# Jabruson/FDN-TIP2025

Hardware: AMD Instinct MI355X
Metric: images/sec, FDN (LPNet->FDN forward) 1280x720 bs=8 fp32 (higher is better)
Workload: dtype f32

## Files before the change

### fdn-tip2025_amd/basicsr/models/archs/FDN_arch.py

```python
import numbers

import numpy as np
import torch
import torch.nn as nn
import torch.nn.functional as F
from einops import rearrange

import fdn_hip
from fdn_hip import ACT_LEAKY, ACT_NONE, ACT_SIGMOID, ops


_Cache = ops.WeightCache


def _w(p):
    return p.detach()


class WithBias_LayerNorm(nn.Module):

    def __init__(self, dim):
        super().__init__()
        self.weight = nn.Parameter(torch.ones(dim))
        self.bias = nn.Parameter(torch.zeros(dim))
# ... 196 lines not shown
    def forward(self, enc, dnc, x_high=None, x_high_p=None, x_img=None):
        n = self.n_feat
        x = ops.conv1x1([enc, dnc], _w(self.conv.weight), _w(self.conv.bias), want_stats=True, cache=(self._c, "c1"))
        x = self.att_channel((x, x_high, x_high_p, x_img))[0]
        wf = self._c.get("w", [self.conv2.weight], lambda: self.conv2.weight.detach()[:n] + self.conv2.weight.detach()[n:])
        bf = self._c.get("b", [self.conv2.bias], lambda: self.conv2.bias.detach()[:n] + self.conv2.bias.detach()[n:])
        return ops.conv1x1(x, wf, bf, cache=(self._c, "c2"), want_stats=True)


class OverlapPatchEmbed(nn.Module):
    def __init__(self, in_c=3, embed_dim=48, bias=False):
        super().__init__()
        self.proj = nn.Conv2d(in_c, embed_dim, kernel_size=3, stride=1, padding=1, bias=bias)

    def forward(self, x):
        return ops.conv2d(x, _w(self.proj.weight), pad=1)


class Downsample(nn.Module):

    def __init__(self, n_feat):
        super().__init__()
        self.body = nn.Sequential(nn.Identity(), nn.Conv2d(n_feat, n_feat * 2, 3, stride=1, padding=1, bias=False))

    def forward(self, x):
        return ops.conv2d(ops.resample(x, ops.RS_BILINEAR_HALF), _w(self.body[1].weight), pad=1)


class Upsample(nn.Module):

    def __init__(self, n_feat):
        super().__init__()
        self.body = nn.Sequential(nn.Identity(), nn.Conv2d(n_feat, n_feat // 2, 3, stride=1, padding=1, bias=False))
        self._c = _Cache()

    def forward(self, x):
        if ops.UPCONV_GATHER:
            return ops.upsample_conv3x3(x, _w(self.body[1].weight), cache=(self._c, "up"))
        return ops.conv2d(ops.resample(x, ops.RS_BILINEAR_X2), _w(self.body[1].weight), pad=1)


class FDformer(nn.Module):

    def __init__(self, inp_channels=3, out_channels=3, dim=48, num_blocks=[6, 6, 12, 8], num_refinement_blocks=4,
                 ffn_expansion_factor=3, bias=False):
        super().__init__()

        def stage(d, n, enc):
            return nn.Sequential(*[TransformerBlock(dim=d, ffn_expansion_factor=ffn_expansion_factor, bias=bias, att=True,
                                                    mode=1 if enc else 2, use_light=enc, use_img=enc) for _ in range(n)])

        self.patch_embed = OverlapPatchEmbed(inp_channels, dim)
        self.encoder_level1 = stage(dim, num_blocks[0], True)
        self.down1_2 = Downsample(dim)
        self.encoder_level2 = stage(dim * 2, num_blocks[1], True)
        self.down2_3 = Downsample(dim * 2)
        self.encoder_level3 = stage(dim * 4, num_blocks[2], True)
        self.decoder_level3 = stage(dim * 4, num_blocks[2], False)
        self.up3_2 = Upsample(dim * 4)
        self.reduce_chan_level2 = nn.Conv2d(dim * 4, dim * 2, kernel_size=1, bias=bias)
        self.decoder_level2 = stage(dim * 2, num_blocks[1], False)
        self.up2_1 = Upsample(dim * 2)
# ... 8 lines not shown
                x_high32=None, x1=None, x2=None, x3=None):
        e1 = self.encoder_level1((self.patch_embed(inp_img), x_high1, x_high12, x1))[0]
        e2 = self.encoder_level2((self.down1_2(e1), x_high2, x_high22, x2))[0]
        e3 = self.encoder_level3((self.down2_3(e2), x_high3, x_high32, x3))[0]
        d3 = self.decoder_level3((e3, x_high3, x_high32, x3))[0]
        d2 = self.fuse2(self.up3_2(d3), e2, x_high2, x_high22, x2)
        d2 = self.decoder_level2((d2, x_high2, x_high22, x2))[0]
        d1 = self.fuse1(self.up2_1(d2), e1, x_high1, x_high12, x1)
        d1 = self.decoder_level1((d1, x_high1, x_high12, x1))[0]
        d1 = self.refinement((d1, x_high1, x_high12, x1))[0]
        res = inp_img if ori_img is None else ori_img
        return ops.conv2d(d1, _w(self.output.weight), pad=1, res=res)


class BasicConv(nn.Module):
    def __init__(self, in_channel, out_channel, kernel_size, stride, bias=True, relu=True, transpose=False):
        super().__init__()
        self.k, self.stride, self.relu, self.transpose = kernel_size, stride, relu, transpose
        if transpose:
            conv = nn.ConvTranspose2d(in_channel, out_channel, kernel_size, padding=kernel_size // 2 - 1, stride=stride, bias=bias)
        else:
            conv = nn.Conv2d(in_channel, out_channel, kernel_size, padding=kernel_size // 2, stride=stride, bias=bias)
        self.main = nn.Sequential(conv)

    def forward(self, x, res=None, res_before_act=False, act=None, post_add=0.0):
        c = self.main[0]
        a = (ACT_LEAKY if self.relu else ACT_NONE) if act is None else act
        if self.transpose:
            return ops.conv_transpose4x4s2(x, _w(c.weight), _w(c.bias), a)
        if self.k == 1 and self.stride == 1:
            return ops.conv1x1(x, _w(c.weight), _w(c.bias), act=a)
        return ops.conv2d(x, _w(c.weight), _w(c.bias), stride=self.stride, pad=self.k // 2, act=a, res=res,
                          res_before_act=res_before_act, post_add=post_add)


class FAM(nn.Module):
    def __init__(self, channel):
        super().__init__()
        self.merge1 = nn.Conv2d(channel * 2, channel, kernel_size=1)
        self.merge2 = nn.Conv2d(channel, channel, kernel_size=3, stride=1, padding=1)

    def forward(self, x1, x2):
        t = ops.conv1x1([x1, x2], _w(self.merge1.weight), _w(self.merge1.bias))
        return ops.conv2d(t, _w(self.merge2.weight), _w(self.merge2.bias), pad=1)


def _mlp2(seq, x):
    t = ops.conv1x1(x, _w(seq[0].weight), _w(seq[0].bias), act=ACT_LEAKY)
    return ops.conv1x1(t, _w(seq[2].weight), _w(seq[2].bias))


def _spectral_mlps(y, process1, process2, H, W):
    z = ops.rfft_rows(y)
    mag, pha = ops.fft_cols_fwd(z, True, True, rd_before=False, fix_real=True)
    if ops.SPECTRAL_MLP_FUSED and mag.shape[1] in ops.SPECTRAL_MLP_C:
        ops.spectral_mlp2(mag, pha, _w(process1[0].weight), _w(process1[0].bias), _w(process1[2].weight), _w(process1[2].bias),
                          _w(process2[0].weight), _w(process2[0].bias), _w(process2[2].weight), _w(process2[2].bias), slope=0.1)
    else:
        mag = _mlp2(process1, mag)
        pha = _mlp2(process2, pha)
    return ops.fft_cols_inv_polar(mag, pha, H, W // 2 + 1)


class FreBlock(nn.Module):
    def __init__(self, nc):
        super().__init__()
        self.fpre = nn.Conv2d(nc, nc, 1, 1, 0)
# ... 26 lines not shown
        self.fourier_out = nn.Conv2d(out_nc, out_nc, 3, 1, 1)
        self._c = _Cache()

    def forward(self, x1, x2, x4):
        return self._rest(ops.conv1x1([x1, x2, x4], _w(self.fpre[0].weight), _w(self.fpre[0].bias)))

    def forward_multires(self, same, up1, up2):
        wfull, bias = _w(self.fpre[0].weight), _w(self.fpre[0].bias)
        n = wfull.shape[0]
        ks = sum(t.shape[1] for t in same)
        k1 = 0 if up1 is None else up1.shape[1]
        w2 = wfull.reshape(n, -1)
        parts = self._c.get("split", [self.fpre[0].weight], lambda: (w2[:, :ks].contiguous(), w2[:, ks:ks + k1].contiguous(), w2[:, ks + k1:].contiguous()))
        acc = ops.conv1x1(up2, parts[2])
        if up1 is not None:
            acc = ops.conv1x1(up1, parts[1], res=ops.resample(acc, ops.RS_NEAREST_X2))
        return self._rest(ops.conv1x1(same, parts[0], bias, res=ops.resample(acc, ops.RS_NEAREST_X2)))

    def _rest(self, y):
        H, W = y.shape[-2:]
        y = ops.dw1x1_pad1(y, _w(self.fpre[1].weight), _w(self.fpre[1].bias))
        zz = _spectral_mlps(y, self.process1, self.process2, H, W)
        xo = ops.irfft_rows(zz, H, W, 2.0 / (H * W))
        return ops.conv2d(xo, _w(self.fourier_out.weight), _w(self.fourier_out.bias), pad=1)


class MAR_archa(nn.Module):
    def __init__(self, use_ratio=True, block=None, apply_ratio=True):
        super().__init__()
        ProcessBlock_ = ProcessBlock if block is None else block
        self.use_ratio = use_ratio
        self.apply_ratio = apply_ratio
        c = 12
        self.Encoder = nn.ModuleList([ProcessBlock_(c), ProcessBlock_(c * 2), ProcessBlock_(c * 4)])
        self.Decoder = nn.ModuleList([ProcessBlock_(c * 4), ProcessBlock_(c * 2), ProcessBlock_(c)])
        self.Convs = nn.ModuleList([BasicConv(c * 4, c * 2, 1, 1, relu=True), BasicConv(c * 2, c, 1, 1, relu=True)])
        self.ConvsOut = nn.ModuleList([BasicConv(c * 4, 3, 3, 1, relu=False), BasicConv(c * 2, 3, 3, 1, relu=False)])
        self.AFFs = nn.ModuleList([fourier_fuse(c * 7, c), fourier_fuse(c * 7, c * 2)])
        self.FAM1 = FAM(c * 4)
        self.f1 = nn.Sequential(nn.Conv2d(3 * 16, c * 4, 1, 1, 0), ProcessBlock_(c * 4))
        self.f2 = nn.Sequential(nn.Conv2d(3 * 4, c * 2, 1, 1, 0), ProcessBlock_(c * 2))
        self.f3 = nn.Sequential(nn.Conv2d(3, c, 1, 1, 0), ProcessBlock_(c))
        self.f3_down = BasicConv(c, c * 2, 3, 2, relu=True)
        self.f2_down = BasicConv(c * 2, c * 4, 3, 2, relu=True)
        self.f2_up = BasicConv(c * 4, c * 2, 4, 2, relu=True, transpose=True)
        self.f3_up = BasicConv(c * 2, c, 4, 2, relu=True, transpose=True)
        self.out = BasicConv(c, 3, 3, 1, relu=False)
# ... 88 lines not shown
```

### fdn-tip2025_amd/basicsr/models/archs/LPNet_arch.py

```python
import torch
import torch.nn as nn
import torch.nn.functional as F
from einops import rearrange

from fdn_hip import ACT_NONE, ACT_RELU, ACT_SIGMOID, ops

from .FDN_arch import _Cache, _w

try:
    from torchvision import transforms
except Exception:
    class _Grayscale:
        def __init__(self, num_output_channels=1):
            self.n = num_output_channels

        def __call__(self, x):
            r, g, b = x.unbind(dim=-3)
            y = (0.2989 * r + 0.587 * g + 0.114 * b).unsqueeze(-3)
            return y if self.n == 1 else y.expand(*x.shape)

    class _Compose:
        def __init__(self, ts):
            self.ts = ts

# ... 23 lines not shown
    def __init__(self, in_channels, filters, stride=1, is_1x1conv=False):
        super().__init__()
        f1, f2, f3 = filters
        self.stride = stride
        self.is_1x1conv = is_1x1conv
        self.conv1 = nn.Sequential(nn.Conv2d(in_channels, f1, 1, stride=stride, bias=False), nn.BatchNorm2d(f1), nn.ReLU())
        self.conv2 = nn.Sequential(nn.Conv2d(f1, f2, 3, stride=1, padding=1, bias=False), nn.BatchNorm2d(f2), nn.ReLU())
        self.conv3 = nn.Sequential(nn.Conv2d(f2, f3, 1, stride=1, bias=False), nn.BatchNorm2d(f3))
        if is_1x1conv:
            self.shortcut = nn.Sequential(nn.Conv2d(in_channels, f3, 1, stride=stride, bias=False), nn.BatchNorm2d(f3))
        self.se = nn.Sequential(nn.AdaptiveAvgPool2d((1, 1)), nn.Conv2d(f3, f3 // 16, 1), nn.ReLU(),
                                nn.Conv2d(f3 // 16, f3, 1), nn.Sigmoid())
        self._c = _Cache()

    def _pw(self, x, seq, name, act, stride):
        w, b = _fold(seq[0], seq[1], self._c, name)
        if stride == 1:
            return ops.conv1x1(x, w, b, act=act)
        return ops.conv2d(x, w, b, stride=stride, pad=0, act=act)

    def forward(self, x):
        y = self._pw(x, self.conv1, "c1", ACT_RELU, self.stride)
        w2, b2 = _fold(self.conv2[0], self.conv2[1], self._c, "c2")
        y = ops.conv2d(y, w2, b2, stride=1, pad=1, act=ACT_RELU)
        y = self._pw(y, self.conv3, "c3", ACT_NONE, 1)
        g = ops.global_avgpool(y)
        g = ops.conv1x1(g, _w(self.se[1].weight), _w(self.se[1].bias), act=ACT_RELU)
        g = ops.conv1x1(g, _w(self.se[3].weight), _w(self.se[3].bias), act=ACT_SIGMOID)
        sc = self._pw(x, self.shortcut, "sc", ACT_NONE, self.stride) if self.is_1x1conv else x
        return ops.se_apply(y, g, sc)


class I_predict_net(nn.Module):

    def __init__(self, c=16):
        super().__init__()
        self.conv1 = nn.Sequential(nn.Conv2d(3, c, kernel_size=7, stride=2, padding=3, bias=False), nn.BatchNorm2d(c),
                                   nn.ReLU(), nn.AvgPool2d(kernel_size=3, stride=2, padding=1))
        self.conv2 = self._make_layer(c, (c, c, 2 * c), 3, 1)
        self.conv3 = self._make_layer(2 * c, (2 * c, 2 * c, 4 * c), 3, 2)
        self.conv4 = self._make_layer(4 * c, (4 * c, 4 * c, 8 * c), 6, 6)
        self.global_average_pool = nn.AdaptiveAvgPool2d((1, 1))
        self.fc = nn.Sequential(nn.Linear(8 * c, 8 * c))
        self.fc2 = nn.Sequential(nn.Linear(8 * c, 1))
        self.sigmoid = nn.Sigmoid()
        self.trans_gray = transforms.Compose([transforms.Grayscale(num_output_channels=1)])
        self._c = _Cache()
# ... 25 lines not shown
```

### fdn-tip2025_amd/csrc/conv3x3.hip

```cpp
#include "common.hpp"
#include <type_traits>

namespace {

constexpr int KC = 32;
using f32x16 = fdn_f32x16;

struct C3Args {
    const float* x; const float* w; const float* bias; const float* res; float* out;
    int B, Cin, H, W, Cout;
    int act, res_before_act; float post_add;
    int tiles_per_img, total_tiles;
    int n0, CoutT;
};

template <int MT, int NW>
__global__ __launch_bounds__(NW * 64, NW == 4 ? 2 : 1) void conv3x3_kernel(C3Args a) {
    extern __shared__ __attribute__((aligned(16))) float Wl[];
    constexpr int NT = NW * 64;
    constexpr int WS = MT * 32 + 1;
    constexpr int CH = KC * WS;
    constexpr int WPT = (KC * MT * 32) / NT;
    const int Cin = a.Cin, N = a.Cout, W = a.W, H = a.H;
    const int Ce = (Cin + 1) & ~1;
// ... 101 lines not shown
                            v = apply_act(v, a.act);
                            if (a.res && !a.res_before_act) v += bload(rr, voff, soff);
                            bstore(v + a.post_add, ro, voff, soff);
                        }
                }
#pragma unroll
                for (int m = 0; m < MT; ++m)
#pragma unroll
                    for (int r = 0; r < 16; ++r) acc[m][r] = 0.f;
            }
            if (nlive) w_stash((step + 1) & 1);
            __syncthreads();
            if (nlive && nc == 0) cur = nxt;
#pragma unroll
            for (int s = 0; s < 16; ++s) xa[s] = xb[s];
            tile = ntile; c = nc; live = nlive;
            ++step;
        }
    }
}

constexpr int TW = 32, CK = 8, HC = TW + 2;

template <int MT, int NW>
__global__ __launch_bounds__(NW * 64, (NW == 4 && MT == 1) ? 2 : 1) void conv3x3_split_kernel(C3Args a, int tiles_x, int tiles_y) {
    extern __shared__ __attribute__((aligned(16))) fdn_u32x4 smem4[];
    constexpr int NT = NW * 64, TH_ = 2 * NW, HR_ = TH_ + 2, NPOS = HR_ * HC;
    constexpr int N = MT * 32, KS5 = 5;
    constexpr int XB = 3 * NPOS, WB = KS5 * 3 * MT * 64;
    constexpr int XE = (NPOS + NT - 1) / NT;
    constexpr int WE = (N * 9 * CK + NT - 1) / NT;
    fdn_u32x4* Xs = smem4;
    fdn_u32x4* Ws = smem4 + 2 * XB;
    const int Cin = a.Cin, H = a.H, W = a.W;
    const unsigned P = (unsigned)H * W, P4 = P * 4u;
    const int tid = threadIdx.x, lane = tid & 63, wave = tid >> 6, kh = lane >> 5, ln = lane & 31;
    const int nchunk = Cin / CK;
    int b, y0, x0;
    {
        const unsigned T = (unsigned)(tiles_x * tiles_y) * a.B;
        const unsigned S0 = xcd_contiguous(blockIdx.x, gridDim.x);
        const unsigned grp = S0 / T, S = S0 - grp * T;
        a.n0 = (int)grp * N;
        const unsigned per = (unsigned)(tiles_x * tiles_y);
        b = (int)(S / per);
        const unsigned t = S - (unsigned)b * per;
        const int ty = (int)(t / (unsigned)tiles_x);
        y0 = ty * TH_;
        x0 = (int)(t - (unsigned)ty * tiles_x) * TW;
    }
    const int nvalid = min(N, a.CoutT - a.n0);
    unsigned xg[XE];
    int xl[XE];
#pragma unroll
    for (int i = 0; i < XE; ++i) {
        const int e = tid + NT * i, r = e / HC, c = e - r * HC;
        const int gy = y0 - 1 + r, gx = x0 - 1 + c;
        const bool in = e < NPOS, ok = in && gy >= 0 && gy < H && gx >= 0 && gx < W;
        xg[i] = ok ? (unsigned)(gy * W + gx) * 4u : 0x80000000u;
        xl[i] = in ? e : -1;
    }
    const rsrc_t rx = mk_rsrc(a.x + (long)b * Cin * P, (unsigned)Cin * P4);
    struct Stage { float xr[XE][CK], wr[WE]; };
    Stage stg[2];
    auto fetch = [&](int c, Stage& sg) __attribute__((always_inline)) {
        float (&xr)[XE][CK] = sg.xr;
        float (&wr)[WE] = sg.wr;
#pragma unroll
        for (int i = 0; i < XE; ++i)
#pragma unroll
            for (int ci = 0; ci < CK; ++ci) xr[i][ci] = bload(rx, xg[i], (unsigned)(c * CK + ci) * P4);
#pragma unroll
        for (int i = 0; i < WE; ++i) {
// ... 57 lines not shown
    auto chunk_step = [&](int c, Stage& mine, const Stage& nxt) __attribute__((always_inline)) {
        const bool more = c + 1 < nchunk;
        if (c + 2 < nchunk) fetch(c + 2, mine);
        const fdn_u32x4* xb = Xs + (c & 1) * XB;
        const fdn_u32x4* wb = Ws + (c & 1) * WB + lane;
#pragma unroll
        for (int s_ = 0; s_ < KS5; ++s_) {
            const fdn_u32x4 b0[3] = {xb[toff[s_]], xb[NPOS + toff[s_]], xb[2 * NPOS + toff[s_]]};
            const fdn_u32x4 b1[3] = {xb[toff[s_] + HC], xb[NPOS + toff[s_] + HC], xb[2 * NPOS + toff[s_] + HC]};
#pragma unroll
            for (int m = 0; m < MT; ++m) {
                const fdn_u32x4 av[3] = {wb[((s_ * 3 + 0) * MT + m) * 64], wb[((s_ * 3 + 1) * MT + m) * 64], wb[((s_ * 3 + 2) * MT + m) * 64]};
                acc[0][m] = fdn_mfma_split6(av, b0, acc[0][m]);
                acc[1][m] = fdn_mfma_split6(av, b1, acc[1][m]);
            }
        }
        if (more) stash((c + 1) & 1, nxt);
        __syncthreads();
    };
    for (int c = 0; c < nchunk; c += 2) {
        chunk_step(c, stg[0], stg[1]);
        if (c + 1 < nchunk) chunk_step(c + 1, stg[1], stg[0]);
    }
    const unsigned nb4 = (unsigned)nvalid * P4;
    const long obase = ((long)b * a.CoutT + a.n0) * P;
    const rsrc_t ro = mk_rsrc(a.out + obase, nb4);
    const rsrc_t rr = mk_rsrc(a.res ? a.res + obase : a.out, a.res ? nb4 : 0u);
    auto epilogue = [&](auto has_act) __attribute__((always_inline)) {
        const int act_ = decltype(has_act)::value ? a.act : (int)FDN_ACT_NONE;
#pragma unroll
        for (int st = 0; st < 2; ++st) {
            const int gy = y0 + row0 + st, gx = x0 + ln;
            const unsigned voff = (gy < H && gx < W) ? (4u * kh * P + (unsigned)(gy * W + gx)) * 4u : 0x80000000u;
#pragma unroll
            for (int m = 0; m < MT; ++m) {
                float rv[16];
                if (a.res) {
#pragma unroll
                    for (int r = 0; r < 16; ++r) {
                        const int nrow = m * 32 + (r & 3) + 8 * (r >> 2);
                        rv[r] = bload(rr, (nrow + 4 * kh < nvalid) ? voff : 0x80000000u, (unsigned)nrow * P4);
                    }
                }
#pragma unroll
                for (int r = 0; r < 16; ++r) {
                    const int nrow = m * 32 + (r & 3) + 8 * (r >> 2);
                    float v = acc[st][m][r];
                    if (a.bias) v += a.bias[a.n0 + min(nrow + 4 * kh, nvalid - 1)];
                    if (a.res && a.res_before_act) v += rv[r];
                    v = apply_act(v, act_);
                    if (a.res && !a.res_before_act) v += rv[r];
                    bstore(v + a.post_add, ro, (nrow + 4 * kh < nvalid) ? voff : 0x80000000u, (unsigned)nrow * P4);
                }
            }
        }
    };
    if (a.act == FDN_ACT_NONE) epilogue(std::false_type{}); else epilogue(std::true_type{});
}

template <int MT, int NW>
int launch_split(const C3Args& a, hipStream_t s) {
    constexpr int N = MT * 32, TH_ = 2 * NW;
    const size_t lds = 2UL * (3UL * (TH_ + 2) * HC + 5UL * 3 * MT * 64) * sizeof(fdn_u32x4);
    auto kern = conv3x3_split_kernel<MT, NW>;
    if (lds > 48 * 1024 && !fdn_allow_dynamic_lds(reinterpret_cast<const void*>(kern), lds)) return FDN_ERR_LAUNCH;
    const int tx = cdiv(a.W, TW), ty = cdiv(a.H, TH_);
    const long total = (long)tx * ty * a.B * cdiv(a.Cout, N);
    if (total > 0x7FFFFFFFL) return FDN_ERR_UNSUPPORTED;
    fdn_note_bf16_launch();
    hipLaunchKernelGGL(kern, dim3((unsigned)total), dim3(NW * 64), lds, s, a, tx, ty);
    return fdn_launch_status();
}

template <int MT, int NW>
int launch(C3Args a, hipStream_t s) {
    const size_t lds = 2UL * KC * (MT * 32 + 1) * sizeof(float);
    a.tiles_per_img = cdiv((long)a.H * a.W, NW * 32);
    a.total_tiles = a.B * a.tiles_per_img;
    auto kern = conv3x3_kernel<MT, NW>;
    const int grid = fdn_persistent_grid(kern, NW * 64, lds, a.total_tiles, {true, 0, 16, 0});
    if (grid < 0) return FDN_ERR_LAUNCH;
    hipLaunchKernelGGL(kern, dim3(grid), dim3(NW * 64), lds, s, a);
    return fdn_launch_status();
}

}

int fdn_conv3x3_mfma(const float* x, const float* w, const float* bias, const float* res, float* out, int B, int Cin, int H,
                     int W, int Cout, int act, int res_before_act, float post_add, hipStream_t s) {
    if (Cin < 2 || Cout < 8) return FDN_ERR_UNSUPPORTED;
    const unsigned long long P4 = 4ull * H * W;
    if ((unsigned long long)(Cin + 2) * P4 > 0xFFFFFFFFull || (unsigned long long)(Cout + 200) * P4 > 0xFFFFFFFFull)
        return FDN_ERR_UNSUPPORTED;
    C3Args a;
    a.x = x; a.w = w; a.bias = bias; a.res = res; a.out = out;
    a.B = B; a.Cin = Cin; a.H = H; a.W = W; a.Cout = Cout;
    a.act = act; a.res_before_act = res_before_act; a.post_add = post_add;
    a.tiles_per_img = a.total_tiles = 0;
    a.n0 = 0; a.CoutT = Cout;
    if (!fdn_matrix_pipe_f32() && Cin % CK == 0 && Cin >= 2 * CK && Cout >= 16)
        return Cout <= 32 ? launch_split<1, 4>(a, s) : launch_split<2, 8>(a, s);
    const int tiles = (Cout + 31) / 32;
    if (tiles == 1) return launch<1, 4>(a, s);
    if (tiles == 2) return launch<2, 4>(a, s);
    if (tiles == 3) return launch<3, 4>(a, s);
    return launch<4, 4>(a, s);
}
```

### fdn-tip2025_amd/fdn_hip/__init__.py

```python
import ctypes
import os

import torch

_HERE = os.path.dirname(os.path.abspath(__file__))
_LIB_PATH = os.path.join(_HERE, "libfdn_hip.so")
_lib = None

ACT_NONE, ACT_LEAKY, ACT_RELU, ACT_SIGMOID, ACT_GELU = 0, 1, 2, 3, 4
PRO_NONE, PRO_LN, PRO_LN3_GATE, PRO_LN_MULADD = 0, 1, 2, 3
EPI_NONE, EPI_RES, EPI_MULADD = 0, 1, 2

c_fp = ctypes.c_void_p


class Conv1x1Desc(ctypes.Structure):
    _fields_ = [
        ("x", c_fp * 3), ("xbs", ctypes.c_long * 3), ("kseg", ctypes.c_int * 3),
        ("w", c_fp), ("bias", c_fp), ("out", c_fp), ("obs", ctypes.c_long),
        ("B", ctypes.c_int), ("K", ctypes.c_int), ("N", ctypes.c_int), ("P", ctypes.c_int),
        ("pro", ctypes.c_int), ("ln_group", ctypes.c_int),
        ("stats", c_fp), ("gamma", c_fp), ("beta", c_fp), ("xb", c_fp), ("xbbs", ctypes.c_long),
        ("act", ctypes.c_int), ("epi", ctypes.c_int),
        ("res", c_fp), ("rbs", ctypes.c_long), ("mul", c_fp), ("add", c_fp), ("mbs", ctypes.c_long),
        ("vec4", ctypes.c_int), ("stats_out", c_fp), ("x_bf16", ctypes.c_int), ("out_bf16", ctypes.c_int), ("wpk", c_fp),
    ]


class FdnHipError(RuntimeError):
    pass


ABI_VERSION = 22
VIDEO_ABI_VERSION = 1
TEMPORAL_ABI_VERSION = 1
VMETRICS_ABI_VERSION = 1
ENSEMBLE_ABI_VERSION = 1


def lib_path():
    return _LIB_PATH


def lib():
    global _lib
    if _lib is None:
        if not os.path.isfile(_LIB_PATH):
            raise ImportError(
                f"{_LIB_PATH} not found: build it with fdn-tip2025_amd/build.sh (hipcc --offload-arch=gfx950). "
                "The FDN path has no CPU fallback.")
        _lib = ctypes.CDLL(_LIB_PATH)
        _declare(_lib)
        if _lib.fdn_abi_version() != ABI_VERSION:
            v = _lib.fdn_abi_version()
            _lib = None
            raise ImportError(f"{_LIB_PATH} has ABI version {v}, this binding needs {ABI_VERSION}: rebuild with build.sh")
        if _lib.fdn_video_abi_version() != VIDEO_ABI_VERSION:
            v = _lib.fdn_video_abi_version()
            _lib = None
            raise ImportError(f"{_LIB_PATH} has video ABI version {v}, this binding needs {VIDEO_ABI_VERSION}: rebuild with build.sh")
        if _lib.fdn_temporal_abi_version() != TEMPORAL_ABI_VERSION:
            v = _lib.fdn_temporal_abi_version()
            _lib = None
            raise ImportError(f"{_LIB_PATH} has temporal ABI version {v}, this binding needs {TEMPORAL_ABI_VERSION}: rebuild with build.sh")
        if _lib.fdn_vmetrics_abi_version() != VMETRICS_ABI_VERSION:
            v = _lib.fdn_vmetrics_abi_version()
            _lib = None
            raise ImportError(f"{_LIB_PATH} has vmetrics ABI version {v}, this binding needs {VMETRICS_ABI_VERSION}: rebuild with build.sh")
        if _lib.fdn_ensemble_abi_version() != ENSEMBLE_ABI_VERSION:
            v = _lib.fdn_ensemble_abi_version()
            _lib = None
            raise ImportError(f"{_LIB_PATH} has ensemble ABI version {v}, this binding needs {ENSEMBLE_ABI_VERSION}: rebuild with build.sh")
    return _lib


def _declare(l, missing_ok=False):
    from ._abi import PROTOTYPES
    from ._abi_video import PROTOTYPES as VIDEO_PROTOTYPES
    from ._abi_temporal import PROTOTYPES as TEMPORAL_PROTOTYPES
    from ._abi_vmetrics import PROTOTYPES as VMETRICS_PROTOTYPES
    from ._abi_ensemble import PROTOTYPES as ENSEMBLE_PROTOTYPES
    kinds = {"P": ctypes.c_void_p, "I": ctypes.c_int, "L": ctypes.c_long, "F": ctypes.c_float, "DESC": ctypes.POINTER(Conv1x1Desc)}
    tables = (PROTOTYPES, VIDEO_PROTOTYPES, TEMPORAL_PROTOTYPES, VMETRICS_PROTOTYPES, ENSEMBLE_PROTOTYPES)
    for name, (ret, sig) in [item for t in tables for item in t.items()]:
        f = getattr(l, name, None) if missing_ok else getattr(l, name)
        if f is None:
            continue
        f.restype = ctypes.c_char_p if ret == "S" else ctypes.c_long if ret == "L" else ctypes.c_int
        f.argtypes = [kinds[k] for k in sig]


def check(code, what):
    if code != 0:
        raise FdnHipError(f"{what}: {lib().fdn_error_string(code).decode()} (code {code})")


def stream():
    return ctypes.c_void_p(torch.cuda.current_stream().cuda_stream)


_storage = "f32"


def set_storage_dtype(name):
    global _storage
    if name not in ("f32", "bf16"):
# ... 62 lines not shown
```

### fdn-tip2025_amd/fdn_hip/lpips.py

```python
import ctypes
import os
from collections.abc import Mapping

import torch

from . import ACT_RELU, FdnHipError, check, lib, ops, stream

SHIFT = (-.030, -.088, -.188)
SCALE = (.458, .448, .450)
LPIPS_PARTS = 1024

ARCH = {
    "vgg": [("conv", 0, 3, 64, 3, 1, 1), ("conv", 2, 64, 64, 3, 1, 1), ("tap",), ("pool", 2, 2),
            ("conv", 5, 64, 128, 3, 1, 1), ("conv", 7, 128, 128, 3, 1, 1), ("tap",), ("pool", 2, 2),
            ("conv", 10, 128, 256, 3, 1, 1), ("conv", 12, 256, 256, 3, 1, 1), ("conv", 14, 256, 256, 3, 1, 1), ("tap",), ("pool", 2, 2),
            ("conv", 17, 256, 512, 3, 1, 1), ("conv", 19, 512, 512, 3, 1, 1), ("conv", 21, 512, 512, 3, 1, 1), ("tap",), ("pool", 2, 2),
            ("conv", 24, 512, 512, 3, 1, 1), ("conv", 26, 512, 512, 3, 1, 1), ("conv", 28, 512, 512, 3, 1, 1), ("tap",)],
    "alex": [("conv", 0, 3, 64, 11, 4, 2), ("tap",), ("pool", 3, 2),
             ("conv", 3, 64, 192, 5, 1, 2), ("tap",), ("pool", 3, 2),
             ("conv", 6, 192, 384, 3, 1, 1), ("tap",),
             ("conv", 8, 384, 256, 3, 1, 1), ("tap",),
             ("conv", 10, 256, 256, 3, 1, 1), ("tap",)],
}

# ... 147 lines not shown
    B = N // 2
    if out is None:
        out = torch.zeros(B, dtype=torch.float64, device=f.device)
    ws = torch.empty(B * LPIPS_PARTS, dtype=torch.float64, device=f.device)
    check(lib().fdn_lpips_layer(ops._flat(f, "f"), ops._flat(w, "w"), _ptr(out), B, C, H, W, int(bool(accumulate)), _ptr(ws), stream()),
          "fdn_lpips_layer")
    return out


class LPIPS:

    def __init__(self, net="vgg", weights=None, lin_weights=None, device=None):
        if weights is None:
            raise FdnHipError("LPIPS: weights are needed (an lpips.LPIPS state_dict, or a torchvision one with lin_weights); none ship here")
        packed = load_weights(net, weights, lin_weights)
        dev = torch.device(device) if device is not None else torch.device("cuda", torch.cuda.current_device())
        if dev.type != "cuda":
            raise FdnHipError(f"LPIPS runs on a ROCm device, got {dev}; there is no CPU fallback")
        if dev.index is None:
            dev = torch.device("cuda", torch.cuda.current_device())
        self.net, self.device = net, dev
        self.convs = [(w.to(dev), b.to(dev)) for w, b in packed["convs"]]
        self.lins = [l.to(dev) for l in packed["lins"]]

    def features(self, x):
        taps, ci = [], 0
        for op in ARCH[self.net]:
            if op[0] == "conv":
                w, b = self.convs[ci]
                ci += 1
                x = ops.conv2d(x, w, b, stride=op[5], pad=op[6], act=ACT_RELU)
            elif op[0] == "pool":
                x = ops.maxpool2d(x, op[1], op[2])
            else:
                taps.append(x)
        return taps

    def _check(self, in0, in1):
        for t in (in0, in1):
            if not torch.is_tensor(t) or t.device != self.device or t.dim() != 4 or t.shape[1] != 3:
                raise FdnHipError(f"LPIPS: inputs are [B,3,H,W] tensors on {self.device}, got "
                                  f"{tuple(t.shape) if torch.is_tensor(t) else type(t).__name__}" + (f" on {t.device}" if torch.is_tensor(t) else ""))
        if in0.shape != in1.shape:
            raise FdnHipError(f"LPIPS: in0 and in1 differ in shape: {tuple(in0.shape)}, {tuple(in1.shape)}")
        tap_sizes(self.net, in0.shape[2], in0.shape[3])

    def _score(self, x, per_layer):
        B = x.shape[0] // 2
        taps = self.features(x)
        out = torch.empty((5, B) if per_layer else (B,), dtype=torch.float64, device=self.device)
        for l, (f, w) in enumerate(zip(taps, self.lins)):
            if per_layer:
                layer(f, w, out[l], accumulate=False)
            else:
# ... 23 lines not shown
```

### fdn-tip2025_amd/fdn_hip/ops.py

```python
import ctypes
import functools

import torch

from . import (ACT_NONE, EPI_MULADD, EPI_NONE, EPI_RES, PRO_LN, PRO_LN3_GATE, PRO_LN_MULADD, PRO_NONE,
               Conv1x1Desc, FdnHipError, check, lib, storage_dtype, stream)

BF16 = torch.bfloat16
ERR_UNSUPPORTED = 4


def _planes(t, what, bf16_ok=False):
    if not t.is_cuda:
        raise FdnHipError(f"{what} must live on a ROCm device (got {t.device}); the FDN path has no CPU fallback")
    if t.dtype != torch.float32 and not (bf16_ok and t.dtype == BF16):
        raise FdnHipError(f"{what} must be float32{' or bfloat16 storage' if bf16_ok else ''} (got {t.dtype})")
    assert t.dim() == 4, what
    _, C, H, W = t.shape
    st = t.stride()
    if not (st[3] == 1 and st[2] == W and st[1] == H * W) and t.numel() > 0:
        raise FdnHipError(f"{what}: channel/row/column dims must be dense (strides {st})")
    return ctypes.c_void_p(t.data_ptr()), (st[0] if t.shape[0] > 1 else C * H * W)


def _flat(t, what, bf16_ok=False):
    if t is None:
        return None
    if not t.is_cuda or not (t.dtype == torch.float32 or (bf16_ok and t.dtype == BF16)) or not t.is_contiguous():
        raise FdnHipError(f"{what} must be a contiguous float32 ROCm tensor")
# ... 509 lines not shown
    guide = pack_guidance(amp, pha, pitch=Wf)
    check(lib().fdn_fft_cols_fcaffn(_flat(z, "z"), _flat(guide, "guide"), _flat(wxa, "wxa"), _flat(wxp, "wxp"), B, C, H, Wf,
                                    stream()), "fdn_fft_cols_fcaffn")
    return z


def fft_cols_fwd(z, want_abs, want_ang, rd_before=False, fix_real=True):
    B, C, H, Wf, _ = z.shape
    oa = torch.empty((B, C, H, Wf), device=z.device, dtype=torch.float32) if want_abs else None
    og = torch.empty((B, C, H, Wf), device=z.device, dtype=torch.float32) if want_ang else None
    check(lib().fdn_fft_cols_fwd(_flat(z, "z"), _flat(oa, "abs"), _flat(og, "ang"), ctypes.c_long(B * C), H, Wf,
                                 int(rd_before), int(fix_real), stream()), "fdn_fft_cols_fwd")
    return oa, og


def fft_cols_inv_polar(mag, pha, H, Wf):
    B, C, Hin, Wfin = mag.shape
    z = torch.empty((B, C, H, Wf, 2), device=mag.device, dtype=torch.float32)
    check(lib().fdn_fft_cols_inv_polar(_flat(mag, "mag"), _flat(pha, "pha"), Hin, Wfin, _flat(z, "z"),
                                       ctypes.c_long(B * C), H, Wf, stream()), "fdn_fft_cols_inv_polar")
    return z


def conv2d(x, w, bias=None, stride=1, pad=0, act=ACT_NONE, res=None, res_before_act=False, post_add=0.0):
    B, Cin, H, W = x.shape
    Cout, _, KH, KW = w.shape
    OH, OW = (H + 2 * pad - KH) // stride + 1, (W + 2 * pad - KW) // stride + 1
    out = torch.empty((B, Cout, OH, OW), device=x.device, dtype=torch.float32)
    check(lib().fdn_conv2d(_flat(x, "x"), _flat(w, "w"), _flat(bias, "bias"), _flat(res, "res"), _flat(out, "out"),
                           B, Cin, H, W, Cout, KH, KW, stride, pad, act, int(res_before_act), ctypes.c_float(post_add),
                           stream()), "fdn_conv2d")
    return out


def maxpool2d(x, k, s):
    B, C, H, W = x.shape
    if H < k or W < k:
        raise FdnHipError(f"maxpool2d: {H}x{W} is smaller than the {k}x{k} window")
    out = torch.empty((B, C, (H - k) // s + 1, (W - k) // s + 1), device=x.device, dtype=torch.float32)
    check(lib().fdn_maxpool2d(_flat(x, "x"), _flat(out, "out"), ctypes.c_long(B * C), H, W, k, s, stream()), "fdn_maxpool2d")
    return out


def conv_transpose4x4s2(x, w, bias, act):
    B, Cin, H, W = x.shape
    Cout = w.shape[1]
    out = torch.empty((B, Cout, 2 * H, 2 * W), device=x.device, dtype=torch.float32)
    check(lib().fdn_conv_transpose4x4s2(_flat(x, "x"), _flat(w, "w"), _flat(bias, "bias"), _flat(out, "out"),
                                        B, Cin, H, W, Cout, act, stream()), "fdn_conv_transpose4x4s2")
    return out

# ... 87 lines not shown
```

Measured before the change: 28.59.

## Add pre-packed bf16-split weight path for 3x3 stride-1 convolutions

Adds a one-time weight packing kernel that splits fp32 3x3 conv weights into three bf16 parts laid out in the exact per-lane MFMA order, cached per module. A new packed conv kernel then loads those weight tiles with wide 128-bit buffer loads straight into LDS, with no per-launch conversion or splitting. Call sites across FDN, LPNet and LPIPS pass cache keys so this path is used when the matrix pipe is not pure f32. The cost is extra device memory for packed weights and a staleness risk if weights change without the cache noticing.

```diff
diff --git a/fdn-tip2025_amd/basicsr/models/archs/FDN_arch.py b/fdn-tip2025_amd/basicsr/models/archs/FDN_arch.py
--- a/fdn-tip2025_amd/basicsr/models/archs/FDN_arch.py
+++ b/fdn-tip2025_amd/basicsr/models/archs/FDN_arch.py
@@ -242,9 +242,10 @@
     def __init__(self, n_feat):
         super().__init__()
         self.body = nn.Sequential(nn.Identity(), nn.Conv2d(n_feat, n_feat * 2, 3, stride=1, padding=1, bias=False))
+        self._c = _Cache()
 
     def forward(self, x):
-        return ops.conv2d(ops.resample(x, ops.RS_BILINEAR_HALF), _w(self.body[1].weight), pad=1)
+        return ops.conv2d(ops.resample(x, ops.RS_BILINEAR_HALF), _w(self.body[1].weight), pad=1, cache=(self._c, "dn"))
 
 
 class Upsample(nn.Module):
@@ -257,7 +258,7 @@
     def forward(self, x):
         if ops.UPCONV_GATHER:
             return ops.upsample_conv3x3(x, _w(self.body[1].weight), cache=(self._c, "up"))
-        return ops.conv2d(ops.resample(x, ops.RS_BILINEAR_X2), _w(self.body[1].weight), pad=1)
+        return ops.conv2d(ops.resample(x, ops.RS_BILINEAR_X2), _w(self.body[1].weight), pad=1, cache=(self._c, "c3"))
 
 
 class FDformer(nn.Module):
@@ -312,6 +313,7 @@
         else:
             conv = nn.Conv2d(in_channel, out_channel, kernel_size, padding=kernel_size // 2, stride=stride, bias=bias)
         self.main = nn.Sequential(conv)
+        self._c = _Cache()
 
     def forward(self, x, res=None, res_before_act=False, act=None, post_add=0.0):
         c = self.main[0]
@@ -321,7 +323,7 @@
         if self.k == 1 and self.stride == 1:
             return ops.conv1x1(x, _w(c.weight), _w(c.bias), act=a)
         return ops.conv2d(x, _w(c.weight), _w(c.bias), stride=self.stride, pad=self.k // 2, act=a, res=res,
-                          res_before_act=res_before_act, post_add=post_add)
+                          res_before_act=res_before_act, post_add=post_add, cache=(self._c, "c"))
 
 
 class FAM(nn.Module):
@@ -329,10 +331,11 @@
         super().__init__()
         self.merge1 = nn.Conv2d(channel * 2, channel, kernel_size=1)
         self.merge2 = nn.Conv2d(channel, channel, kernel_size=3, stride=1, padding=1)
+        self._c = _Cache()
 
     def forward(self, x1, x2):
         t = ops.conv1x1([x1, x2], _w(self.merge1.weight), _w(self.merge1.bias))
-        return ops.conv2d(t, _w(self.merge2.weight), _w(self.merge2.bias), pad=1)
+        return ops.conv2d(t, _w(self.merge2.weight), _w(self.merge2.bias), pad=1, cache=(self._c, "m2"))
 
 
 def _mlp2(seq, x):
@@ -405,7 +408,7 @@
         y = ops.dw1x1_pad1(y, _w(self.fpre[1].weight), _w(self.fpre[1].bias))
         zz = _spectral_mlps(y, self.process1, self.process2, H, W)
         xo = ops.irfft_rows(zz, H, W, 2.0 / (H * W))
-        return ops.conv2d(xo, _w(self.fourier_out.weight), _w(self.fourier_out.bias), pad=1)
+        return ops.conv2d(xo, _w(self.fourier_out.weight), _w(self.fourier_out.bias), pad=1, cache=(self._c, "fo"))
 
 
 class MAR_archa(nn.Module):
diff --git a/fdn-tip2025_amd/basicsr/models/archs/LPNet_arch.py b/fdn-tip2025_amd/basicsr/models/archs/LPNet_arch.py
--- a/fdn-tip2025_amd/basicsr/models/archs/LPNet_arch.py
+++ b/fdn-tip2025_amd/basicsr/models/archs/LPNet_arch.py
@@ -69,7 +69,7 @@
     def forward(self, x):
         y = self._pw(x, self.conv1, "c1", ACT_RELU, self.stride)
         w2, b2 = _fold(self.conv2[0], self.conv2[1], self._c, "c2")
-        y = ops.conv2d(y, w2, b2, stride=1, pad=1, act=ACT_RELU)
+        y = ops.conv2d(y, w2, b2, stride=1, pad=1, act=ACT_RELU, cache=(self._c, "c2"))
         y = self._pw(y, self.conv3, "c3", ACT_NONE, 1)
         g = ops.global_avgpool(y)
         g = ops.conv1x1(g, _w(self.se[1].weight), _w(self.se[1].bias), act=ACT_RELU)
diff --git a/fdn-tip2025_amd/csrc/conv3x3.hip b/fdn-tip2025_amd/csrc/conv3x3.hip
--- a/fdn-tip2025_amd/csrc/conv3x3.hip
+++ b/fdn-tip2025_amd/csrc/conv3x3.hip
@@ -1,4 +1,6 @@
 #include "common.hpp"
+#include "../../include/fdn_conv3x3.h"
+#include <cstdint>
 #include <type_traits>
 
 namespace {
@@ -147,6 +149,60 @@
 
 constexpr int TW = 32, CK = 8, HC = TW + 2;
 
+template <int N, int TH_>
+__device__ __forceinline__ void split_place(C3Args& a, int tiles_x, int tiles_y, int& b, int& y0, int& x0) {
+    const unsigned T = (unsigned)(tiles_x * tiles_y) * a.B;
+    const unsigned S0 = xcd_contiguous(blockIdx.x, gridDim.x);
+    const unsigned grp = S0 / T, S = S0 - grp * T;
+    a.n0 = (int)grp * N;
+    const unsigned per = (unsigned)(tiles_x * tiles_y);
+    b = (int)(S / per);
+    const unsigned t = S - (unsigned)b * per;
+    const int ty = (int)(t / (unsigned)tiles_x);
+    y0 = ty * TH_;
+    x0 = (int)(t - (unsigned)ty * tiles_x) * TW;
+}
+
+template <int MT>
+__device__ __forceinline__ void split_epilogue(const C3Args& a, const f32x16 (&acc)[2][MT], int b, int y0, int x0, int row0, int nvalid, int kh, int ln) {
+    const int H = a.H, W = a.W;
+    const unsigned P = (unsigned)H * W, P4 = P * 4u;
+    const unsigned nb4 = (unsigned)nvalid * P4;
+    const long obase = ((long)b * a.CoutT + a.n0) * P;
+    const rsrc_t ro = mk_rsrc(a.out + obase, nb4);
+    const rsrc_t rr = mk_rsrc(a.res ? a.res + obase : a.out, a.res ? nb4 : 0u);
+    auto epilogue = [&](auto has_act) __attribute__((always_inline)) {
+        const int act_ = decltype(has_act)::value ? a.act : (int)FDN_ACT_NONE;
+#pragma unroll
+        for (int st = 0; st < 2; ++st) {
+            const int gy = y0 + row0 + st, gx = x0 + ln;
+            const unsigned voff = (gy < H && gx < W) ? (4u * kh * P + (unsigned)(gy * W + gx)) * 4u : 0x80000000u;
+#pragma unroll
+            for (int m = 0; m < MT; ++m) {
+                float rv[16];
+                if (a.res) {
+#pragma unroll
+                    for (int r = 0; r < 16; ++r) {
+                        const int nrow = m * 32 + (r & 3) + 8 * (r >> 2);
+                        rv[r] = bload(rr, (nrow + 4 * kh < nvalid) ? voff : 0x80000000u, (unsigned)nrow * P4);
+                    }
+                }
+#pragma unroll
+                for (int r = 0; r < 16; ++r) {
+                    const int nrow = m * 32 + (r & 3) + 8 * (r >> 2);
+                    float v = acc[st][m][r];
+                    if (a.bias) v += a.bias[a.n0 + min(nrow + 4 * kh, nvalid - 1)];
+                    if (a.res && a.res_before_act) v += rv[r];
+                    v = apply_act(v, act_);
+                    if (a.res && !a.res_before_act) v += rv[r];
+                    bstore(v + a.post_add, ro, (nrow + 4 * kh < nvalid) ? voff : 0x80000000u, (unsigned)nrow * P4);
+                }
+            }
+        }
+    };
+    if (a.act == FDN_ACT_NONE) epilogue(std::false_type{}); else epilogue(std::true_type{});
+}
+
 template <int MT, int NW>
 __global__ __launch_bounds__(NW * 64, (NW == 4 && MT == 1) ? 2 : 1) void conv3x3_split_kernel(C3Args a, int tiles_x, int tiles_y) {
     extern __shared__ __attribute__((aligned(16))) fdn_u32x4 smem4[];
@@ -162,18 +218,7 @@
     const int tid = threadIdx.x, lane = tid & 63, wave = tid >> 6, kh = lane >> 5, ln = lane & 31;
     const int nchunk = Cin / CK;
     int b, y0, x0;
-    {
-        const unsigned T = (unsigned)(tiles_x * tiles_y) * a.B;
-        const unsigned S0 = xcd_contiguous(blockIdx.x, gridDim.x);
-        const unsigned grp = S0 / T, S = S0 - grp * T;
-        a.n0 = (int)grp * N;
-        const unsigned per = (unsigned)(tiles_x * tiles_y);
-        b = (int)(S / per);
-        const unsigned t = S - (unsigned)b * per;
-        const int ty = (int)(t / (unsigned)tiles_x);
-        y0 = ty * TH_;
-        x0 = (int)(t - (unsigned)ty * tiles_x) * TW;
-    }
+    split_place<N, TH_>(a, tiles_x, tiles_y, b, y0, x0);
     const int nvalid = min(N, a.CoutT - a.n0);
     unsigned xg[XE];
     int xl[XE];
@@ -277,40 +322,7 @@
         chunk_step(c, stg[0], stg[1]);
         if (c + 1 < nchunk) chunk_step(c + 1, stg[1], stg[0]);
     }
-    const unsigned nb4 = (unsigned)nvalid * P4;
-    const long obase = ((long)b * a.CoutT + a.n0) * P;
-    const rsrc_t ro = mk_rsrc(a.out + obase, nb4);
-    const rsrc_t rr = mk_rsrc(a.res ? a.res + obase : a.out, a.res ? nb4 : 0u);
-    auto epilogue = [&](auto has_act) __attribute__((always_inline)) {
-        const int act_ = decltype(has_act)::value ? a.act : (int)FDN_ACT_NONE;
-#pragma unroll
-        for (int st = 0; st < 2; ++st) {
-            const int gy = y0 + row0 + st, gx = x0 + ln;
-            const unsigned voff = (gy < H && gx < W) ? (4u * kh * P + (unsigned)(gy * W + gx)) * 4u : 0x80000000u;
-#pragma unroll
-            for (int m = 0; m < MT; ++m) {
-                float rv[16];
-                if (a.res) {
-#pragma unroll
-                    for (int r = 0; r < 16; ++r) {
-                        const int nrow = m * 32 + (r & 3) + 8 * (r >> 2);
-                        rv[r] = bload(rr, (nrow + 4 * kh < nvalid) ? voff : 0x80000000u, (unsigned)nrow * P4);
-                    }
-                }
-#pragma unroll
-                for (int r = 0; r < 16; ++r) {
-                    const int nrow = m * 32 + (r & 3) + 8 * (r >> 2);
-                    float v = acc[st][m][r];
-                    if (a.bias) v += a.bias[a.n0 + min(nrow + 4 * kh, nvalid - 1)];
-                    if (a.res && a.res_before_act) v += rv[r];
-                    v = apply_act(v, act_);
-                    if (a.res && !a.res_before_act) v += rv[r];
-                    bstore(v + a.post_add, ro, (nrow + 4 * kh < nvalid) ? voff : 0x80000000u, (unsigned)nrow * P4);
-                }
-            }
-        }
-    };
-    if (a.act == FDN_ACT_NONE) epilogue(std::false_type{}); else epilogue(std::true_type{});
+    split_epilogue<MT>(a, acc, b, y0, x0, row0, nvalid, kh, ln);
 }
 
 template <int MT, int NW>
@@ -326,6 +338,165 @@
     hipLaunchKernelGGL(kern, dim3((unsigned)total), dim3(NW * 64), lds, s, a, tx, ty);
     return fdn_launch_status();
 }
+
+constexpr int pk_cells(int MT) { return 16 * MT * 64; }
+
+template <int MT>
+__global__ __launch_bounds__(256) void conv3x3_pack_kernel(const float* __restrict__ w, fdn_u32x4* __restrict__ wpk, int Cin, int Cout, long cells) {
+    constexpr int WBP = pk_cells(MT);
+    const long u = (long)blockIdx.x * 256 + threadIdx.x;
+    if (u >= cells) return;
+    const int nchunk = Cin / CK;
+    const int q = (int)(u % WBP), gc = (int)(u / WBP), c = gc % nchunk, g = gc / nchunk;
+    const int lane = q & 63, m = (q >> 6) % MT, sp = q / (64 * MT), part = sp % 3, s_ = sp / 3;
+    const int tap = 2 * s_ + (lane >> 5), n = g * (MT * 32) + m * 32 + (lane & 31);
+    unsigned short h[CK];
+#pragma unroll
+    for (int ci = 0; ci < CK; ++ci) {
+        const float v = (s_ < 5 && tap < 9 && n < Cout) ? w[((long)n * Cin + c * CK + ci) * 9 + tap] : 0.f;
+        const float w1 = fdn_trunc_bf16(v), r1 = v - w1, w2 = fdn_trunc_bf16(r1), w3 = r1 - w2;
+        h[ci] = (unsigned short)(__float_as_uint(part == 0 ? w1 : part == 1 ? w2 : w3) >> 16);
+    }
+    wpk[u] = fdn_u32x4{h[0] | (unsigned)h[1] << 16, h[2] | (unsigned)h[3] << 16, h[4] | (unsigned)h[5] << 16, h[6] | (unsigned)h[7] << 16};
+}
+
+template <int MT, int NW>
+__global__ __launch_bounds__(NW * 64, (NW == 4 && MT == 1) ? 2 : 1) void conv3x3_packed_kernel(C3Args a, int tiles_x, int tiles_y) {
+    extern __shared__ __attribute__((aligned(16))) fdn_u32x4 smem4[];
+    constexpr int NT = NW * 64, TH_ = 2 * NW, HR_ = TH_ + 2, NPOS = HR_ * HC;
+    constexpr int N = MT * 32, KS5 = 5;
+    constexpr int XB = 3 * NPOS, WBP = pk_cells(MT);
+    constexpr int XE = (NPOS + NT - 1) / NT;
+    constexpr int WE = WBP / NT;
+    static_assert(WBP % NT == 0, "every thread moves the same number of weight cells");
+    fdn_u32x4* Xs = smem4;
+    fdn_u32x4* Ws = smem4 + 2 * XB;
+    const int Cin = a.Cin, H = a.H, W = a.W;
+    const unsigned P = (unsigned)H * W, P4 = P * 4u;
+    const int tid = threadIdx.x, lane = tid & 63, wave = tid >> 6, kh = lane >> 5, ln = lane & 31;
+    const int nchunk = Cin / CK;
+    int b, y0, x0;
+    split_place<N, TH_>(a, tiles_x, tiles_y, b, y0, x0);
+    const int nvalid = min(N, a.CoutT - a.n0);
+    unsigned xg[XE];
+    int xl[XE];
+#pragma unroll
+    for (int i = 0; i < XE; ++i) {
+        const int e = tid + NT * i, r = e / HC, c = e - r * HC;
+        const int gy = y0 - 1 + r, gx = x0 - 1 + c;
+        const bool in = e < NPOS, ok = in && gy >= 0 && gy < H && gx >= 0 && gx < W;
+        xg[i] = ok ? (unsigned)(gy * W + gx) * 4u : 0x80000000u;
+        xl[i] = in ? e : -1;
+    }
+    const float* xbase = a.x + (long)b * Cin * P;
+    constexpr unsigned CHB = (unsigned)WBP * 16u;
+    const char* wbase = reinterpret_cast<const char*>(a.w) + (long)(a.n0 / N) * nchunk * CHB;
+    struct Stage { float xr[XE][CK]; };
+    Stage stg[2];
+    fdn_u32x4 wr[WE];
+    auto fetch_w = [&](int c) __attribute__((always_inline)) {
+        const rsrc_t rw = mk_rsrc(wbase, c < nchunk ? (unsigned)nchunk * CHB : 0u);
+#pragma unroll
+        for (int i = 0; i < WE; ++i) wr[i] = __builtin_amdgcn_raw_buffer_load_b128(rw, (unsigned)(tid + NT * i) * 16u, (unsigned)min(c, nchunk - 1) * CHB, 0);
+    };
+    auto fetch = [&](int c, Stage& sg) __attribute__((always_inline)) {
+        const rsrc_t rx = mk_rsrc(xbase, c < nchunk ? (unsigned)Cin * P4 : 0u);
+        const int cc = min(c, nchunk - 1);
+#pragma unroll
+        for (int i = 0; i < XE; ++i)
+#pragma unroll
+            for (int ci = 0; ci < CK; ++ci) sg.xr[i][ci] = bload(rx, xg[i], (unsigned)(cc * CK + ci) * P4);
+    };
+    auto stash = [&](int buf, const Stage& sg) __attribute__((always_inline)) {
+        fdn_u32x4* xd = Xs + buf * XB;
+#pragma unroll
+        for (int i = 0; i < XE; ++i) {
+            fdn_u32x4 p1, p2, p3;
+#pragma unroll
+            for (int j = 0; j < 4; ++j) {
+                unsigned u1, u2, u3;
+                fdn_split3(sg.xr[i][2 * j], sg.xr[i][2 * j + 1], u1, u2, u3);
+                p1[j] = u1; p2[j] = u2; p3[j] = u3;
+            }
+            if (xl[i] >= 0) {
+                xd[xl[i]] = p1;
+                xd[NPOS + xl[i]] = p2;
+                xd[2 * NPOS + xl[i]] = p3;
+            }
+        }
+        fdn_u32x4* wd = Ws + buf * WBP + tid;
+#pragma unroll
+        for (int i = 0; i < WE; ++i) wd[NT * i] = wr[i];
+    };
+    f32x16 acc[2][MT];
+#pragma unroll
+    for (int st = 0; st < 2; ++st)
+#pragma unroll
+        for (int m = 0; m < MT; ++m)
+#pragma unroll
+            for (int r = 0; r < 16; ++r) acc[st][m][r] = 0.f;
+
+    fetch_w(0);
+    fetch(0, stg[0]);
+    fetch(1, stg[1]);
+    stash(0, stg[0]);
+    __syncthreads();
+    const int row0 = 2 * wave;
+    int toff[KS5];
+#pragma unroll
+    for (int s_ = 0; s_ < KS5; ++s_) {
+        const int tap = min(2 * s_ + kh, 8), dy = tap / 3, dx = tap - dy * 3;
+        toff[s_] = (row0 + dy) * HC + ln + dx;
+    }
+    auto chunk_step = [&](int c, Stage& mine, const Stage& nxt) __attribute__((always_inline)) {
+        fetch_w(c + 1);
+        fetch(c + 2, mine);
+        const fdn_u32x4* xb = Xs + (c & 1) * XB;
+        const fdn_u32x4* wb = Ws + (c & 1) * WBP + lane;
+#pragma unroll
+        for (int s_ = 0; s_ < KS5; ++s_) {
+            const fdn_u32x4 b0[3] = {xb[toff[s_]], xb[NPOS + toff[s_]], xb[2 * NPOS + toff[s_]]};
+            const fdn_u32x4 b1[3] = {xb[toff[s_] + HC], xb[NPOS + toff[s_] + HC], xb[2 * NPOS + toff[s_] + HC]};
+#pragma unroll
+            for (int m = 0; m < MT; ++m) {
+                const fdn_u32x4 av[3] = {wb[((s_ * 3 + 0) * MT + m) * 64], wb[((s_ * 3 + 1) * MT + m) * 64], wb[((s_ * 3 + 2) * MT + m) * 64]};
+                acc[0][m] = fdn_mfma_split6(av, b0, acc[0][m]);
+                acc[1][m] = fdn_mfma_split6(av, b1, acc[1][m]);
+            }
+        }
+        stash((c + 1) & 1, nxt);
+        __syncthreads();
+    };
+    auto pairs = [&](int c, Stage& s0, Stage& s1) __attribute__((always_inline)) {
+        for (; c < nchunk; c += 2) {
+            chunk_step(c, s0, s1);
+            chunk_step(c + 1, s1, s0);
+        }
+    };
+    if (nchunk & 1) {
+        chunk_step(0, stg[0], stg[1]);
+        pairs(1, stg[1], stg[0]);
+    } else {
+        pairs(0, stg[0], stg[1]);
+    }
+    split_epilogue<MT>(a, acc, b, y0, x0, row0, nvalid, kh, ln);
+}
+
+template <int MT, int NW>
+int launch_packed(const C3Args& a, hipStream_t s) {
+    constexpr int N = MT * 32, TH_ = 2 * NW;
+    const size_t lds = 2UL * (3UL * (TH_ + 2) * HC + pk_cells(MT)) * sizeof(fdn_u32x4);
+    auto kern = conv3x3_packed_kernel<MT, NW>;
+    if (lds > 48 * 1024 && !fdn_allow_dynamic_lds(reinterpret_cast<const void*>(kern), lds)) return FDN_ERR_LAUNCH;
+    const int tx = cdiv(a.W, TW), ty = cdiv(a.H, TH_);
+    const long total = (long)tx * ty * a.B * cdiv(a.Cout, N);
+    if (total > 0x7FFFFFFFL) return FDN_ERR_UNSUPPORTED;
+    fdn_note_bf16_launch();
+    hipLaunchKernelGGL(kern, dim3((unsigned)total), dim3(NW * 64), lds, s, a, tx, ty);
+    return fdn_launch_status();
+}
+
+inline int packed_mt(int Cin, int Cout) { return (Cin % CK == 0 && Cin >= 2 * CK && Cout >= 16) ? (Cout <= 32 ? 1 : 2) : 0; }
 
 template <int MT, int NW>
 int launch(C3Args a, hipStream_t s) {
@@ -361,3 +532,41 @@
     if (tiles == 3) return launch<3, 4>(a, s);
     return launch<4, 4>(a, s);
 }
+
+extern "C" int fdn_conv3x3_abi_version(void) { return 1; }
+
+extern "C" long fdn_conv3x3_pack_bytes(int Cin, int Cout) {
+    const int mt = (Cin > 0 && Cout > 0) ? packed_mt(Cin, Cout) : 0;
+    return mt ? (long)cdiv(Cout, 32 * mt) * (Cin / CK) * pk_cells(mt) * 16L : 0L;
+}
+
+extern "C" int fdn_conv3x3_pack(const float* w, int Cin, int Cout, void* wpk, fdn_stream_t stream) {
+    FDN_CHECK_ARG(w && wpk && Cin > 0 && Cout > 0);
+    const int mt = packed_mt(Cin, Cout);
+    if (!mt) return FDN_ERR_UNSUPPORTED;
+    const long cells = fdn_conv3x3_pack_bytes(Cin, Cout) / 16;
+    if (cells > 0x7FFFFFFFL) return FDN_ERR_UNSUPPORTED;
+    hipStream_t s = static_cast<hipStream_t>(stream);
+    if (mt == 1) hipLaunchKernelGGL(conv3x3_pack_kernel<1>, dim3(cdiv(cells, 256)), dim3(256), 0, s, w, static_cast<fdn_u32x4*>(wpk), Cin, Cout, cells);
+    else hipLaunchKernelGGL(conv3x3_pack_kernel<2>, dim3(cdiv(cells, 256)), dim3(256), 0, s, w, static_cast<fdn_u32x4*>(wpk), Cin, Cout, cells);
+    return fdn_launch_status();
+}
+
+extern "C" int fdn_conv3x3_packed(const float* x, const void* wpk, const float* bias, const float* res, float* out, int B, int Cin, int H, int W,
+                                  int Cout, int act, int res_before_act, float post_add, fdn_stream_t stream) {
+    FDN_CHECK_ARG(x && wpk && out && B > 0 && Cin > 0 && Cout > 0 && H > 0 && W > 0);
+    FDN_CHECK_ARG((reinterpret_cast<uintptr_t>(wpk) & 15) == 0);
+    const int mt = packed_mt(Cin, Cout);
+    if (!mt || fdn_matrix_pipe_f32()) return FDN_ERR_UNSUPPORTED;
+    const unsigned long long P4 = 4ull * H * W;
+    if ((unsigned long long)(Cin + 2) * P4 > 0xFFFFFFFFull || (unsigned long long)(Cout + 200) * P4 > 0xFFFFFFFFull) return FDN_ERR_UNSUPPORTED;
+    if (fdn_conv3x3_pack_bytes(Cin, Cout) > 0x7FFFFFFFL) return FDN_ERR_UNSUPPORTED;
+    C3Args a;
+    a.x = x; a.w = static_cast<const float*>(wpk); a.bias = bias; a.res = res; a.out = out;
+    a.B = B; a.Cin = Cin; a.H = H; a.W = W; a.Cout = Cout;
+    a.act = act; a.res_before_act = res_before_act; a.post_add = post_add;
+    a.tiles_per_img = a.total_tiles = 0;
+    a.n0 = 0; a.CoutT = Cout;
+    hipStream_t s = static_cast<hipStream_t>(stream);
+    return mt == 1 ? launch_packed<1, 4>(a, s) : launch_packed<2, 8>(a, s);
+}
diff --git a/fdn-tip2025_amd/fdn_hip/__init__.py b/fdn-tip2025_amd/fdn_hip/__init__.py
--- a/fdn-tip2025_amd/fdn_hip/__init__.py
+++ b/fdn-tip2025_amd/fdn_hip/__init__.py
@@ -36,6 +36,7 @@
 TEMPORAL_ABI_VERSION = 1
 VMETRICS_ABI_VERSION = 1
 ENSEMBLE_ABI_VERSION = 1
+CONV3X3_ABI_VERSION = 1
 
 
 def lib_path():
@@ -71,6 +72,10 @@
             v = _lib.fdn_ensemble_abi_version()
             _lib = None
             raise ImportError(f"{_LIB_PATH} has ensemble ABI version {v}, this binding needs {ENSEMBLE_ABI_VERSION}: rebuild with build.sh")
+        if _lib.fdn_conv3x3_abi_version() != CONV3X3_ABI_VERSION:
+            v = _lib.fdn_conv3x3_abi_version()
+            _lib = None
+            raise ImportError(f"{_LIB_PATH} has conv3x3 ABI version {v}, this binding needs {CONV3X3_ABI_VERSION}: rebuild with build.sh")
     return _lib
 
 
@@ -80,8 +85,9 @@
     from ._abi_temporal import PROTOTYPES as TEMPORAL_PROTOTYPES
     from ._abi_vmetrics import PROTOTYPES as VMETRICS_PROTOTYPES
     from ._abi_ensemble import PROTOTYPES as ENSEMBLE_PROTOTYPES
+    from ._abi_conv3x3 import PROTOTYPES as CONV3X3_PROTOTYPES
     kinds = {"P": ctypes.c_void_p, "I": ctypes.c_int, "L": ctypes.c_long, "F": ctypes.c_float, "DESC": ctypes.POINTER(Conv1x1Desc)}
-    tables = (PROTOTYPES, VIDEO_PROTOTYPES, TEMPORAL_PROTOTYPES, VMETRICS_PROTOTYPES, ENSEMBLE_PROTOTYPES)
+    tables = (PROTOTYPES, VIDEO_PROTOTYPES, TEMPORAL_PROTOTYPES, VMETRICS_PROTOTYPES, ENSEMBLE_PROTOTYPES, CONV3X3_PROTOTYPES)
     for name, (ret, sig) in [item for t in tables for item in t.items()]:
         f = getattr(l, name, None) if missing_ok else getattr(l, name)
         if f is None:
diff --git a/fdn-tip2025_amd/fdn_hip/_abi_conv3x3.py b/fdn-tip2025_amd/fdn_hip/_abi_conv3x3.py
--- /dev/null
+++ b/fdn-tip2025_amd/fdn_hip/_abi_conv3x3.py
@@ -0,0 +1,14 @@
+
+PROTOTYPES = {
+    "fdn_conv3x3_abi_version": ("I", []),
+    "fdn_conv3x3_pack_bytes": ("L", ['I', 'I']),
+    "fdn_conv3x3_pack": ("I", ['P', 'I', 'I', 'P', 'P']),
+    "fdn_conv3x3_packed": ("I", ['P', 'P', 'P', 'P', 'P', 'I', 'I', 'I', 'I', 'I', 'I', 'I', 'F', 'P']),
+}
+
+ARG_NAMES = {
+    "fdn_conv3x3_abi_version": [],
+    "fdn_conv3x3_pack_bytes": ['Cin', 'Cout'],
+    "fdn_conv3x3_pack": ['w', 'Cin', 'Cout', 'wpk', 'stream'],
+    "fdn_conv3x3_packed": ['x', 'wpk', 'bias', 'res', 'out', 'B', 'Cin', 'H', 'W', 'Cout', 'act', 'res_before_act', 'post_add', 'stream'],
+}
diff --git a/fdn-tip2025_amd/fdn_hip/lpips.py b/fdn-tip2025_amd/fdn_hip/lpips.py
--- a/fdn-tip2025_amd/fdn_hip/lpips.py
+++ b/fdn-tip2025_amd/fdn_hip/lpips.py
@@ -193,14 +193,15 @@
         self.net, self.device = net, dev
         self.convs = [(w.to(dev), b.to(dev)) for w, b in packed["convs"]]
         self.lins = [l.to(dev) for l in packed["lins"]]
+        self._c = ops.WeightCache()
 
     def features(self, x):
         taps, ci = [], 0
         for op in ARCH[self.net]:
             if op[0] == "conv":
                 w, b = self.convs[ci]
+                x = ops.conv2d(x, w, b, stride=op[5], pad=op[6], act=ACT_RELU, cache=(self._c, f"c{ci}"))
                 ci += 1
-                x = ops.conv2d(x, w, b, stride=op[5], pad=op[6], act=ACT_RELU)
             elif op[0] == "pool":
                 x = ops.maxpool2d(x, op[1], op[2])
             else:
diff --git a/fdn-tip2025_amd/fdn_hip/ops.py b/fdn-tip2025_amd/fdn_hip/ops.py
--- a/fdn-tip2025_amd/fdn_hip/ops.py
+++ b/fdn-tip2025_amd/fdn_hip/ops.py
@@ -4,7 +4,7 @@
 import torch
 
 from . import (ACT_NONE, EPI_MULADD, EPI_NONE, EPI_RES, PRO_LN, PRO_LN3_GATE, PRO_LN_MULADD, PRO_NONE,
-               Conv1x1Desc, FdnHipError, check, lib, storage_dtype, stream)
+               Conv1x1Desc, FdnHipError, check, lib, matrix_pipe, storage_dtype, stream)
 
 BF16 = torch.bfloat16
 ERR_UNSUPPORTED = 4
@@ -560,11 +560,29 @@
     return z
 
 
-def conv2d(x, w, bias=None, stride=1, pad=0, act=ACT_NONE, res=None, res_before_act=False, post_add=0.0):
+def conv3x3_pack(w):
+    Cout, Cin = w.shape[:2]
+    nbytes = lib().fdn_conv3x3_pack_bytes(Cin, Cout)
+    if not nbytes:
+        return None
+    wpk = torch.empty(nbytes, device=w.device, dtype=torch.uint8)
+    check(lib().fdn_conv3x3_pack(_flat(w, "w"), Cin, Cout, ctypes.c_void_p(wpk.data_ptr()), stream()), "fdn_conv3x3_pack")
+    return wpk
+
+
+def conv2d(x, w, bias=None, stride=1, pad=0, act=ACT_NONE, res=None, res_before_act=False, post_add=0.0, cache=None):
     B, Cin, H, W = x.shape
     Cout, _, KH, KW = w.shape
     OH, OW = (H + 2 * pad - KH) // stride + 1, (W + 2 * pad - KW) // stride + 1
     out = torch.empty((B, Cout, OH, OW), device=x.device, dtype=torch.float32)
+    if (cache is not None and (KH, KW, stride, pad) == (3, 3, 1, 1) and matrix_pipe() != "f32"
+            and lib().fdn_conv3x3_pack_bytes(Cin, Cout) > 0):
+        wpk = cache[0].get(cache[1] + ":pk3", [w], lambda: conv3x3_pack(w))
+        rc = lib().fdn_conv3x3_packed(_flat(x, "x"), ctypes.c_void_p(wpk.data_ptr()), _flat(bias, "bias"), _flat(res, "res"), _flat(out, "out"),
+                                      B, Cin, H, W, Cout, act, int(res_before_act), ctypes.c_float(post_add), stream())
+        if rc != ERR_UNSUPPORTED:
+            check(rc, "fdn_conv3x3_packed")
+            return out
     check(lib().fdn_conv2d(_flat(x, "x"), _flat(w, "w"), _flat(bias, "bias"), _flat(res, "res"), _flat(out, "out"),
                            B, Cin, H, W, Cout, KH, KW, stride, pad, act, int(res_before_act), ctypes.c_float(post_add),
                            stream()), "fdn_conv2d")
diff --git a/include/fdn_conv3x3.h b/include/fdn_conv3x3.h
--- /dev/null
+++ b/include/fdn_conv3x3.h
@@ -0,0 +1,22 @@
+#ifndef FDN_CONV3X3_H
+#define FDN_CONV3X3_H
+
+#include "fdn_hip.h"
+
+#ifdef __cplusplus
+extern "C" {
+#endif
+
+int fdn_conv3x3_abi_version(void);
+
+long fdn_conv3x3_pack_bytes(int Cin, int Cout);
+
+int fdn_conv3x3_pack(const float* w, int Cin, int Cout, void* wpk, fdn_stream_t stream);
+
+int fdn_conv3x3_packed(const float* x, const void* wpk, const float* bias, const float* res, float* out, int B, int Cin, int H, int W,
+                       int Cout, int act, int res_before_act, float post_add, fdn_stream_t stream);
+
+#ifdef __cplusplus
+}
+#endif
+#endif
```

Result: no change. 28.58 (-0.0%).
